# hse-cs/probaforms

Hardware: AMD Instinct MI355X
Metric: RealNVP samples/sec (fit+sample) (higher is better)
Workload: dtype f32 (first Linear of the s/t nets on 3-term split-bf16 MFMA, float32-level accuracy in: the training kernel's forward phase, sampling, log-prob; everything else f32); 1 GPU; C2: RealNVP n=1000000/GPU d=16 cond=4 L=8 hidden=(128,); one step = one fit epoch over the rank's 1000000 rows (16 batches of 65536 rows per rank incl. the ragged one: loss+grad+Adam each) + sampling 1000000 rows (counter-based prior draw inside the inverse kernel); global_batch=65536, rank_batch=65536, batch_mode=per-rank batch fixed (default): the global batch grows with N, parallelism=dp1, rccl_ranks=0

## Files before the change

### probaforms_amd/csrc/rnvp_mfma_layer.h

```cpp
#pragma once
#include "rnvp_mfma.h"

namespace rnvp {
namespace mfma {

using f4 = __attribute__((ext_vector_type(4))) float;

__device__ __forceinline__ f4 mfma16(float a, float b, f4 c) {
    return __builtin_amdgcn_mfma_f32_16x16x4f32(a, b, c, 0, 0, 0);
}

__device__ __forceinline__ f4 mfma4(float a, float b, f4 c) {
    return __builtin_amdgcn_mfma_f32_4x4x1f32(a, b, c, 0, 0, 0);
}

__device__ __forceinline__ float swap_add32(float x, float y) {
    const auto r = __builtin_amdgcn_permlane32_swap(__float_as_uint(x), __float_as_uint(y), false, false);
    return __uint_as_float(r[0]) + __uint_as_float(r[1]);
}
__device__ __forceinline__ float swap_add16(float x, float y) {
    const auto r = __builtin_amdgcn_permlane16_swap(__float_as_uint(x), __float_as_uint(y), false, false);
    return __uint_as_float(r[0]) + __uint_as_float(r[1]);
}

#ifndef RNVP_ABLATE
#define RNVP_ABLATE 0
#endif
#ifdef RNVP_NO_X4
constexpr bool kUseX4 = false;
#else
constexpr bool kUseX4 = true;
#endif

constexpr float kTanhScale = 2.8853900817779268f;
using f2 = __attribute__((ext_vector_type(2))) float;

__device__ __forceinline__ f4 tanh4(f4 u) {
    if (RNVP_ABLATE & 8) return u * 0.5f;
    f2 e0, e1;
    e0[0] = __builtin_amdgcn_exp2f(u[0]); e0[1] = __builtin_amdgcn_exp2f(u[1]);
    e1[0] = __builtin_amdgcn_exp2f(u[2]); e1[1] = __builtin_amdgcn_exp2f(u[3]);
    e0 = e0 + 1.0f; e1 = e1 + 1.0f;
    f2 r0, r1;
    r0[0] = __builtin_amdgcn_rcpf(e0[0]); r0[1] = __builtin_amdgcn_rcpf(e0[1]);
    r1[0] = __builtin_amdgcn_rcpf(e1[0]); r1[1] = __builtin_amdgcn_rcpf(e1[1]);
    r0 = __builtin_elementwise_fma(r0, f2{-2.0f, -2.0f}, f2{1.0f, 1.0f});
    r1 = __builtin_elementwise_fma(r1, f2{-2.0f, -2.0f}, f2{1.0f, 1.0f});
    return f4{r0[0], r0[1], r1[0], r1[1]};
}

template <int ACT> __device__ __forceinline__ f4 act4(f4 u) {
    if constexpr (ACT == 0) return tanh4(u);
    return f4{fmaxf(u[0], 0.f), fmaxf(u[1], 0.f), fmaxf(u[2], 0.f), fmaxf(u[3], 0.f)};
}
template <int ACT> __device__ __forceinline__ f4 dact4(f4 hv) {
    if constexpr (ACT == 0) return 1.0f - hv * hv;
    return f4{hv[0] > 0.f ? 1.f : 0.f, hv[1] > 0.f ? 1.f : 0.f, hv[2] > 0.f ? 1.f : 0.f, hv[3] > 0.f ? 1.f : 0.f};
}

typedef const __attribute__((address_space(1))) f4 *gf4_ptr;
__device__ __forceinline__ gf4_ptr opaque(const float *p) {
    asm volatile("" : "+v"(p));
    return (gf4_ptr)p;
}

template <int NF, int CQ, bool WITH_X = true>
__device__ __forceinline__ void load_row(const float *x, const float *__restrict__ c, int64_t src,
                                         int d, int cd, bool full, int q, float (&xr)[2 * NF],
                                         float (&cr)[CQ > 0 ? CQ : 1]) {
    if (full) {
        if constexpr (WITH_X) {
            const float *xp = x + src * (8 * NF) + q * 2 * NF;
#pragma unroll
            for (int v = 0; v < 2 * NF; v += 4) {
                const f4 t = *reinterpret_cast<const f4 *>(xp + v);
                xr[v] = t[0]; xr[v + 1] = t[1]; xr[v + 2] = t[2]; xr[v + 3] = t[3];
            }
        }
        if (CQ > 0) {
            const float *cp = c + src * (4 * CQ) + q * CQ;
#pragma unroll
            for (int v = 0; v < CQ; ++v) cr[v] = cp[v];
        } else {
            cr[0] = 0.f;
        }
    } else {
        if constexpr (WITH_X) {
#pragma unroll
            for (int v = 0; v < 2 * NF; ++v) {
                const int j = q * 2 * NF + v;
                xr[v] = (j < d) ? x[src * d + j] : 0.f;
            }
        }
#pragma unroll
        for (int v = 0; v < (CQ > 0 ? CQ : 1); ++v) {
            const int j = q * CQ + v;
            cr[v] = (CQ > 0 && j < cd) ? c[src * cd + j] : 0.f;
        }
    }
}

template <int NF>
__device__ __forceinline__ void store_row(float *out, int64_t row, int d, bool full, int q, const float (&xr)[2 * NF]) {
    if (full) {
        float *op = out + row * (8 * NF) + q * 2 * NF;
#pragma unroll
        for (int v = 0; v < 2 * NF; v += 4) {
            f4 t;
            t[0] = xr[v]; t[1] = xr[v + 1]; t[2] = xr[v + 2]; t[3] = xr[v + 3];
            *reinterpret_cast<f4 *>(op + v) = t;
        }
    } else {
#pragma unroll
        for (int v = 0; v < 2 * NF; ++v) {
            const int j = q * 2 * NF + v;
            if (j < d) out[row * d + j] = xr[v];
// ... 185 lines not shown
    }
    auto gemm2 = [&](const St &c, const f4 (&hv)[R]) {
#pragma unroll
        for (int o = 0; o < OTL; ++o)
#pragma unroll
            for (int rho = 0; rho < 4; ++rho)
#pragma unroll
                for (int rt = 0; rt < R; ++rt) out[rt][OT0 + o] = mfma16(c.a2c[o][rho], hv[rt][rho], out[rt][OT0 + o]);
    };
    auto step = [&](const St &c, St &nx, int t) {
        const int t2 = (t + 2 < last) ? t + 2 : last;
#pragma unroll
        for (int k4 = 0; k4 < K4; ++k4) nx.a1n[k4] = *opaque(pA1 + ((size_t)t2 * K4 + k4) * 256);
        nx.b1n = *opaque(pB1 + t2 * 16);
#pragma unroll
        for (int o = 0; o < OTL; ++o) nx.a2c[o] = *opaque(pA2 + ((size_t)(t + 1) * OTL + o) * 256);
        __builtin_amdgcn_sched_barrier(0);
        f4 hv[R];
        constexpr int RB = (R % 2 == 0) ? 2 : 1;
#pragma unroll
        for (int r0 = 0; r0 < R; r0 += RB) {
#pragma unroll
            for (int u = 0; u < RB; ++u) nx.acc[r0 + u] = c.b1n;
            if constexpr (BX) {
#pragma unroll
                for (int i = 0; i < K4; ++i)
#pragma unroll
                    for (int u = 0; u < RB; ++u) nx.acc[r0 + u] = mfma32(c.a1n[i], bin[r0 + u][i], nx.acc[r0 + u]);
            } else {
#pragma unroll
                for (int kk = 0; kk < NF + CQ; ++kk)
#pragma unroll
                    for (int u = 0; u < RB; ++u)
                        nx.acc[r0 + u] = mfma16(c.a1n[kk >> 2][kk & 3], in_op<NF, CQ, PC, R>(xr, cr, r0 + u, kk), nx.acc[r0 + u]);
            }
#pragma unroll
            for (int u = 0; u < RB; ++u) hv[r0 + u] = act4<ACT>(c.acc[r0 + u]);
            __builtin_amdgcn_sched_barrier(0);
        }
        gemm2(c, hv);
        __builtin_amdgcn_sched_barrier(0);
    };
    auto finish = [&](const St &c) {
        f4 hv[R];
#pragma unroll
        for (int rt = 0; rt < R; ++rt) hv[rt] = act4<ACT>(c.acc[rt]);
        gemm2(c, hv);
    };
    int t = 0;
    for (; t + 1 < last; t += 2) { step(s0, s1, t); step(s1, s0, t + 1); }
    if (t < last) { step(s0, s1, t); finish(s1); } else finish(s0);
}

template <int CQ, int R, int PC, int NET, int ACT, bool BX = false>
__device__ __forceinline__ void run_tiles_x4(const float *__restrict__ W, const Geo &g, int lane, int tile0,
                                             int ntiles, const float (&xr)[R][4],
                                             const float (&cr)[R][CQ > 0 ? CQ : 1], f4 (&outx)[R][4],
                                             const f4 (*bin)[SplitDims<2, CQ>::NI1] = nullptr,
                                             const TilePre<2, CQ> *pre = nullptr) {
    constexpr int NF = 2;
    constexpr int K4 = G1Dims<NF, CQ, BX>::NA;
    const int q = lane >> 4;
    const float *pA1 = W + (BX ? g.oA1S : g.oA1) + ((size_t)tile0 * K4 * 64 + lane) * 4;
    const float *pB1 = W + g.oB1 + ((size_t)tile0 * 4 + q) * 4;
    const float *pA2 = W + g.oA2X + ((size_t)tile0 * 2 * 64 + lane) * 4;
    const int last = ntiles - 1;
    struct St { f4 a1n[K4], b1n, a2c[2], acc[R]; };
    St s0, s1;
    {
        f4 a1c[K4], b1c;
        bool have = false;
        if constexpr (!BX) {
            if (pre) {
                have = true;
#pragma unroll
                for (int k4 = 0; k4 < K4; ++k4) { a1c[k4] = pre->a1c[k4]; s0.a1n[k4] = pre->a1n[k4]; }
                b1c = pre->b1c; s0.b1n = pre->b1n;
                s0.a2c[0] = pre->a2c[0]; s0.a2c[1] = pre->a2c[1];
            }
        }
        if (!have) {
#pragma unroll
        for (int k4 = 0; k4 < K4; ++k4) a1c[k4] = *reinterpret_cast<const f4 *>(pA1 + k4 * 256);
        b1c = *reinterpret_cast<const f4 *>(pB1);
#pragma unroll
        for (int o = 0; o < 2; ++o) s0.a2c[o] = *reinterpret_cast<const f4 *>(pA2 + o * 256);
        const int t1 = last < 1 ? last : 1;
#pragma unroll
        for (int k4 = 0; k4 < K4; ++k4) s0.a1n[k4] = *opaque(pA1 + ((size_t)t1 * K4 + k4) * 256);
        s0.b1n = *opaque(pB1 + t1 * 16);
        }
#pragma unroll
        for (int rt = 0; rt < R; ++rt) s0.acc[rt] = gemm1_any<NF, CQ, PC, R, BX>(a1c, b1c, xr, cr, bin, rt);
    }
    auto gemm2 = [&](const St &c, const f4 (&hv)[R]) {
#pragma unroll
        for (int rho = 0; rho < 4; ++rho)
#pragma unroll
            for (int o = 0; o < 2; ++o)
#pragma unroll
                for (int rt = 0; rt < R; ++rt)
                    outx[rt][2 * NET + o] = mfma4(c.a2c[o][rho], hv[rt][rho], outx[rt][2 * NET + o]);
    };
    auto step = [&](const St &c, St &nx, int t) {
        const int t2 = (t + 2 < last) ? t + 2 : last;
#pragma unroll
        for (int k4 = 0; k4 < K4; ++k4) nx.a1n[k4] = *opaque(pA1 + ((size_t)t2 * K4 + k4) * 256);
        nx.b1n = *opaque(pB1 + t2 * 16);
#pragma unroll
        for (int o = 0; o < 2; ++o) nx.a2c[o] = *opaque(pA2 + ((size_t)(t + 1) * 2 + o) * 256);
        __builtin_amdgcn_sched_barrier(0);
        f4 hv[R];
        constexpr int RB = (R % 2 == 0) ? 2 : 1;
#pragma unroll
        for (int r0 = 0; r0 < R; r0 += RB) {
#pragma unroll
            for (int u = 0; u < RB; ++u) nx.acc[r0 + u] = c.b1n;
            if constexpr (BX) {
#pragma unroll
                for (int i = 0; i < K4; ++i)
#pragma unroll
                    for (int u = 0; u < RB; ++u) nx.acc[r0 + u] = mfma32(c.a1n[i], bin[r0 + u][i], nx.acc[r0 + u]);
            } else {
#pragma unroll
                for (int kk = 0; kk < NF + CQ; ++kk)
#pragma unroll
                    for (int u = 0; u < RB; ++u)
                        nx.acc[r0 + u] = mfma16(c.a1n[kk >> 2][kk & 3], in_op<NF, CQ, PC, R>(xr, cr, r0 + u, kk), nx.acc[r0 + u]);
            }
#pragma unroll
            for (int u = 0; u < RB; ++u) hv[r0 + u] = act4<ACT>(c.acc[r0 + u]);
            __builtin_amdgcn_sched_barrier(0);
        }
        gemm2(c, hv);
        __builtin_amdgcn_sched_barrier(0);
    };
    auto finish = [&](const St &c) {
        f4 hv[R];
#pragma unroll
        for (int rt = 0; rt < R; ++rt) hv[rt] = act4<ACT>(c.acc[rt]);
        gemm2(c, hv);
    };
    int t = 0;
    for (; t + 1 < last; t += 2) { step(s0, s1, t); step(s1, s0, t + 1); }
    if (t < last) { step(s0, s1, t); finish(s1); } else finish(s0);
}

__device__ __forceinline__ void reduce_scatter_x4(const f4 (&part)[4], float (&tv)[2], float (&sv)[2]) {
#pragma unroll
    for (int net = 0; net < 2; ++net) {
        float s4[4];
#pragma unroll
        for (int i = 0; i < 4; ++i) s4[i] = swap_add32(part[2 * net][i], part[2 * net + 1][i]);
        const float f0 = swap_add16(s4[0], s4[2]), f1 = swap_add16(s4[1], s4[3]);
        if (net == 0) { tv[0] = f0; tv[1] = f1; } else { sv[0] = f0; sv[1] = f1; }
    }
}

template <int NF, int CQ, int R, int PC, int MODE, int ACT, bool BX = false>
__device__ __forceinline__ void layer_forward(const float *__restrict__ W, const Geo &g, int lane,
                                              float (&xr)[R][2 * NF], const float (&cr)[R][CQ > 0 ? CQ : 1],
                                              float (&ld)[R], float *__restrict__ scr) {
    using D = FwdDims<NF, CQ>;
// ... 15 lines not shown
        for (int rt = 0; rt < R; ++rt) {
            float tv[2], sv[2];
            reduce_scatter_x4(outx[rt], tv, sv);
            out[rt][0] = f4{tv[0], tv[1], sv[0], sv[1]} + bias2;
        }
    } else {
#pragma unroll
        for (int ot = 0; ot < NT2; ++ot) {
            const f4 b = (ot == 0) ? bias2 : *reinterpret_cast<const f4 *>(W + g.oB2 + (ot * 4 + q) * 4);
#pragma unroll
            for (int rt = 0; rt < R; ++rt) out[rt][ot] = b;
        }
        if (NF >= 4) {
            run_tiles<NF, CQ, R, PC, 0, ACT, BX>(W, g, lane, 0, g.HT, xr, cr, out, bin);
            run_tiles<NF, CQ, R, PC, (NF >= 4 ? OTL : 0), ACT, BX>(W, g, lane, g.HT, g.HT, xr, cr, out, bin);
        } else {
            run_tiles<NF, CQ, R, PC, 0, ACT, BX>(W, g, lane, 0, 2 * g.HT, xr, cr, out, bin);
        }
    }
#pragma unroll
    for (int rt = 0; rt < R; ++rt) {
#pragma unroll
        for (int f = 0; f < NF; ++f) {
            float tv, sv;
            if (NF >= 4) { tv = out[rt][f >> 2][f & 3]; sv = out[rt][(NF >= 4 ? OTL : 0) + (f >> 2)][f & 3]; }
            else { tv = out[rt][0][f & 1]; sv = out[rt][0][2 + (f & 1)]; }
            const int e = 2 * f + 1 - PC;
            if (MODE == 1) {
                xr[rt][e] = (xr[rt][e] - tv) * expf(-sv);
            } else {
                const float es = expf(sv), xv = xr[rt][e];
                if (MODE == 2) {
                    scr[((rt * 2 * NF) + f) * 64 + lane] = xv;
                    scr[((rt * 2 * NF) + NF + f) * 64 + lane] = es;
                }
                xr[rt][e] = fmaf(xv, es, tv);
                ld[rt] += sv;
            }
        }
    }
}

template <int NF, int CQ, int R, int PC, int MODE, int ACT, bool BX = false>
__device__ __forceinline__ void layer_forward_ns(const float *__restrict__ W, const Geo &g, int lane, int role,
                                                 float *xown, const float *xother, float (&xr)[R][2 * NF],
                                                 const float (&cr)[R][CQ > 0 ? CQ : 1], float (&ld)[R],
                                                 float *__restrict__ scr) {
    using D = FwdDims<NF, CQ>;
    constexpr int OTL = D::OTL, NT2 = D::NT2;
    const int q = lane >> 4;
    f4 bin[BX ? R : 1][SplitDims<NF, CQ>::NI1];
    if constexpr (BX) build_bin<NF, CQ, PC, R>(xr, cr, bin);
    float own[R][NF];
    if constexpr (NF == 2 && kUseX4) {
        const f4 bias2 = *reinterpret_cast<const f4 *>(W + g.oB2 + q * 4);
        f4 outx[R][4];
#pragma unroll
        for (int rt = 0; rt < R; ++rt)
#pragma unroll
            for (int u = 0; u < 4; ++u) outx[rt][u] = f4{0.f, 0.f, 0.f, 0.f};
        if (role == 0) {
            run_tiles_x4<CQ, R, PC, 0, ACT, BX>(W, g, lane, 0, g.HT, xr, cr, outx, bin);
#pragma unroll
            for (int rt = 0; rt < R; ++rt) {
                float s4[4];
#pragma unroll
                for (int i = 0; i < 4; ++i) s4[i] = swap_add32(outx[rt][0][i], outx[rt][1][i]);
                own[rt][0] = swap_add16(s4[0], s4[2]) + bias2[0];
                own[rt][1] = swap_add16(s4[1], s4[3]) + bias2[1];
            }
        } else {
            run_tiles_x4<CQ, R, PC, 1, ACT, BX>(W, g, lane, g.HT, g.HT, xr, cr, outx, bin);
#pragma unroll
            for (int rt = 0; rt < R; ++rt) {
                float s4[4];
#pragma unroll
                for (int i = 0; i < 4; ++i) s4[i] = swap_add32(outx[rt][2][i], outx[rt][3][i]);
                own[rt][0] = swap_add16(s4[0], s4[2]) + bias2[2];
                own[rt][1] = swap_add16(s4[1], s4[3]) + bias2[3];
            }
        }
    } else {
        f4 out[R][NT2];
#pragma unroll
        for (int ot = 0; ot < NT2; ++ot) {
            const f4 b = *reinterpret_cast<const f4 *>(W + g.oB2 + (ot * 4 + q) * 4);
#pragma unroll
            for (int rt = 0; rt < R; ++rt) out[rt][ot] = b;
        }
        if (role == 0) {
            run_tiles<NF, CQ, R, PC, 0, ACT, BX>(W, g, lane, 0, g.HT, xr, cr, out, bin);
#pragma unroll
            for (int rt = 0; rt < R; ++rt)
#pragma unroll
                for (int f = 0; f < NF; ++f) own[rt][f] = out[rt][f >> 2][f & 3];
        } else {
            run_tiles<NF, CQ, R, PC, (NF >= 4 ? OTL : 0), ACT, BX>(W, g, lane, g.HT, g.HT, xr, cr, out, bin);
#pragma unroll
            for (int rt = 0; rt < R; ++rt)
#pragma unroll
                for (int f = 0; f < NF; ++f) own[rt][f] = out[rt][(NF >= 4 ? OTL : 0) + (f >> 2)][(f & 3) + (NF >= 4 ? 0 : 2)];
        }
    }
#pragma unroll
    for (int rt = 0; rt < R; ++rt)
#pragma unroll
        for (int f = 0; f < NF; ++f) xown[(rt * NF + f) * 64 + lane] = own[rt][f];
    __syncthreads();
#pragma unroll
    for (int rt = 0; rt < R; ++rt) {
#pragma unroll
        for (int f = 0; f < NF; ++f) {
            const float oth = xother[(rt * NF + f) * 64 + lane];
            const float tv = role == 0 ? own[rt][f] : oth, sv = role == 0 ? oth : own[rt][f];
            const int e = 2 * f + 1 - PC;
            if (MODE == 1) {
                xr[rt][e] = (xr[rt][e] - tv) * expf(-sv);
            } else {
                const float es = expf(sv), xv = xr[rt][e];
                if (MODE == 2) {
                    if (role == 0) scr[((rt * 2 * NF) + f) * 64 + lane] = xv;
                    else scr[((rt * 2 * NF) + NF + f) * 64 + lane] = es;
                }
                xr[rt][e] = fmaf(xv, es, tv);
                ld[rt] += sv;
            }
        }
    }
}

constexpr int kTsWaves = 8, kTsSlices = 4;
template <int NF, int CQ, int R, int PC, int MODE, int ACT>
__device__ __forceinline__ void layer_forward_ts(const float *__restrict__ W, const Geo &g, int lane, int wave, int tile0,
                                                 int nt, float *red, float (&xr)[R][2 * NF],
                                                 const float (&cr)[R][CQ > 0 ? CQ : 1], float (&ld)[R],
                                                 float *__restrict__ scr, const float *__restrict__ Wnext,
                                                 TilePre<NF, CQ> &pre, bool use_pre) {
    using D = FwdDims<NF, CQ>;
    constexpr int OTL = D::OTL, NT2 = D::NT2;
    const int q = lane >> 4, net = wave >> 2;
    float b2t[NF], b2s[NF];
#pragma unroll
    for (int f = 0; f < NF; ++f) {
        if (NF >= 4) {
            b2t[f] = W[g.oB2 + ((f >> 2) * 4 + q) * 4 + (f & 3)];
            b2s[f] = W[g.oB2 + ((OTL + (f >> 2)) * 4 + q) * 4 + (f & 3)];
        } else {
            b2t[f] = W[g.oB2 + q * 4 + (f & 1)];
            b2s[f] = W[g.oB2 + q * 4 + 2 + (f & 1)];
        }
    }
    float own[R][NF];
    if constexpr (NF == 2 && kUseX4) {
        f4 outx[R][4];
#pragma unroll
        for (int rt = 0; rt < R; ++rt)
#pragma unroll
            for (int u = 0; u < 4; ++u) outx[rt][u] = f4{0.f, 0.f, 0.f, 0.f};
        if (nt > 0) {
            if (net == 0) run_tiles_x4<CQ, R, PC, 0, ACT>(W, g, lane, tile0, nt, xr, cr, outx, nullptr, use_pre ? &pre : nullptr);
            else run_tiles_x4<CQ, R, PC, 1, ACT>(W, g, lane, g.HT + tile0, nt, xr, cr, outx, nullptr, use_pre ? &pre : nullptr);
// ... 63 lines not shown
```

### probaforms_amd/csrc/rnvp_mfma_train_dev.h

```cpp
#pragma once
#include <atomic>

#include "rnvp_mfma_layer.h"

#ifndef RNVP_WPE
#define RNVP_WPE 2
#endif

namespace rnvp {
namespace mfma {

struct TrainPlan {
    int glayer_floats;
    size_t lds_bytes;
    int RMAX;
    size_t scratch_per_wave;
};
struct PartialLayout { int glayer_floats, w2c; };

namespace {

constexpr int kAblate = RNVP_ABLATE;
#ifdef RNVP_STAMP
#define STAMP(var) do { __builtin_amdgcn_sched_barrier(0); var = __builtin_readcyclecounter(); __builtin_amdgcn_sched_barrier(0); } while (0)
// ... 62 lines not shown
        return (w2c<NS>() ? gimg<NS>(R) : NT2 * 16 * kTS) + 16 * SIN + 2 * (R >= 4 ? 2 : R) * 16 * kTS;
    }
};

template <int NF, int CQ, int R> struct BwdPre {
    static constexpr int K4 = Dims<NF, CQ>::K4, OTL = Dims<NF, CQ>::OTL, NGI = (NF == 2 && kUseX4) ? 2 : Dims<NF, CQ>::MTI;
    float sx[R][NF], se[R][NF];
    f4 a1[K4], b1, a2t[OTL], a1t[NGI];
};
template <int NF, int CQ, int R>
__device__ __forceinline__ void load_bwd_pre(const float *__restrict__ W, const Geo &g, int lane, const float *__restrict__ scr,
                                             int net, int ht_lo, BwdPre<NF, CQ, R> &p) {
    using P = BwdPre<NF, CQ, R>;
    constexpr int K4 = P::K4, OTL = P::OTL, NGI = P::NGI;
    constexpr bool X4 = (NF == 2) && kUseX4;
    const int q = lane >> 4, HT = g.HT;
#pragma unroll
    for (int rt = 0; rt < R; ++rt)
#pragma unroll
        for (int f = 0; f < NF; ++f) {
            p.sx[rt][f] = scr[((rt * 2 * NF) + f) * 64 + lane];
            p.se[rt][f] = scr[((rt * 2 * NF) + NF + f) * 64 + lane];
        }
    const float *pA1 = W + g.oA1 + ((size_t)net * HT * K4 * 64 + lane) * 4;
    const float *pB1 = W + g.oB1 + ((size_t)net * HT * 4 + q) * 4;
    const float *pA2T = W + g.oA2T + ((size_t)net * HT * OTL * 64 + lane) * 4;
    const float *pA1T = W + (X4 ? g.oA1X : g.oA1T) + ((size_t)net * HT * NGI * 64 + lane) * 4;
#pragma unroll
    for (int k4 = 0; k4 < K4; ++k4) p.a1[k4] = *opaque(pA1 + ((size_t)ht_lo * K4 + k4) * 256);
    p.b1 = *opaque(pB1 + ht_lo * 16);
#pragma unroll
    for (int o = 0; o < OTL; ++o) p.a2t[o] = *opaque(pA2T + ((size_t)ht_lo * OTL + o) * 256);
#pragma unroll
    for (int m = 0; m < NGI; ++m) p.a1t[m] = *opaque(pA1T + ((size_t)ht_lo * NGI + m) * 256);
}

template <int NF, int CQ, int R, int PC, int NS, int ACT, int WV = kWaves>
__device__ __forceinline__ void layer_bwd(const float *__restrict__ W, const Geo &g, int lane, int wave,
                                          float (&xr)[R][2 * NF], const float (&cr)[R][CQ > 0 ? CQ : 1],
                                          float (&gy)[R][2 * NF], const float (&gld)[R],
                                          const float *__restrict__ scr, float *lds, float *tb,
                                          float *gp_layer, bool first, Stamps &stp, float *xown,
                                          const float *xother, int tile_lo, int tile_hi,
                                          BwdPre<NF, CQ, R> &pre_ref, bool use_pre, const float *__restrict__ Wprev = nullptr,
                                          const float *__restrict__ scr_prev = nullptr, FlushSync *fs = nullptr) {
    BwdPre<NF, CQ, R> *const pre = &pre_ref;
    constexpr bool TS = NS == 2;
    unsigned long long t0 = 0; (void)t0;
    STAMP(t0);
    using D = Dims<NF, CQ>;
    constexpr int KS1 = D::KS1, K4 = D::K4, OTL = D::OTL, NT2 = D::NT2, KP4 = D::KP4, NTI = D::NTI,
                  MTI = D::MTI, KSP = D::KSP, SIN = D::SIN;
    const int q = lane >> 4, r = lane & 15, tid = wave * 64 + lane;
    const int role = NS ? (wave >> 2) : 0;
    const int HT = g.HT;
    const int ht_lo = TS ? tile_lo : 0, ht_hi = TS ? tile_hi : HT;
    constexpr bool W2C = D::template w2c<NS>();
    constexpr int FT = D::FT, SLOT = D::template slot<NS>(), TBLK = D::template tblk<NS>(), GS = D::GS;
    constexpr bool TFW = kWideTFlush && NS == 0 && WV == 8 && FT >= 2 && FT % 2 == 0;
    constexpr bool TF = (kNsTFlush && NS == 1 && FT >= 2 && FT % 2 == 0 && WV == 4) || TFW;
    constexpr int FT2 = FT / 2 > 0 ? FT / 2 : 1;
    const int netblock = HT * TBLK;
    float *slot = lds + wave * SLOT;
    float *bufG = tb;
    float *bufI = tb + (W2C ? D::template gimg<NS>(R) : NT2 * 16 * kTS);
    float *bufH = bufI + 16 * SIN;
    f4 go[R][NT2];
#pragma unroll
    for (int rt = 0; rt < R; ++rt) {
#pragma unroll
        for (int f = 0; f < NF; ++f) {
            const float sx = (TS && use_pre) ? pre->sx[rt][f] : scr[((rt * 2 * NF) + f) * 64 + lane];
            const float se = (TS && use_pre) ? pre->se[rt][f] : scr[((rt * 2 * NF) + NF + f) * 64 + lane];
            const int e = 2 * f + 1 - PC;
            const float gyv = gy[rt][e];
            const float gt = gyv;
            const float gs = fmaf(gyv * sx, se, gld[rt]);
            gy[rt][e] = gyv * se;
            xr[rt][e] = sx;
            if (NF >= 4) { go[rt][f >> 2][f & 3] = gt; go[rt][(NF >= 4 ? OTL : 0) + (f >> 2)][f & 3] = gs; }
            else { go[rt][0][f & 1] = gt; go[rt][0][2 + (f & 1)] = gs; }
        }
    }
    f4 gb2[NT2];
#pragma unroll
    for (int ot = 0; ot < NT2; ++ot) {
        gb2[ot] = go[0][ot];
#pragma unroll
        for (int rt = 1; rt < R; ++rt) gb2[ot] += go[rt][ot];
    }
    float goT[R][NT2][4], inT[R][NTI][4];
#pragma unroll
    for (int rt = 0; rt < R; ++rt) {
        if constexpr (W2C && NS == 0) {
            float *gp = bufG + (rt * 16 + r) * GS + 4 * (q & 1) + (q >> 1);
            wave_lds_fence();
            gp[0] = go[rt][0][0]; gp[2] = go[rt][0][1];
            gp[R * 16 * GS] = go[rt][0][2]; gp[R * 16 * GS + 2] = go[rt][0][3];
        } else if constexpr (W2C) {
            const float v0 = role ? go[rt][0][2] : go[rt][0][0], v1 = role ? go[rt][0][3] : go[rt][0][1];
            float *gp = bufG + (rt * 16 + r) * GS + 4 * (q & 1) + (q >> 1);
            wave_lds_fence();
            gp[0] = v0; gp[2] = v1;
        } else {
#pragma unroll
            for (int ot = 0; ot < NT2; ++ot) transpose16(bufG + ot * 16 * kTS, go[rt][ot], lane, goT[rt][ot]);
        }
        wave_lds_fence();
#pragma unroll
        for (int k4 = 0; k4 < KP4; ++k4) {
            f4 v;
#pragma unroll
            for (int u = 0; u < 4; ++u) {
                const int kk = 4 * k4 + u;
                v[u] = (kk < KS1) ? in_op<NF, CQ, PC, R>(xr, cr, rt, kk < KS1 ? kk : 0)
                                  : (kk == KS1 ? (q == 0 ? 1.0f : 0.0f) : 0.0f);
            }
            *reinterpret_cast<f4 *>(bufI + r * SIN + q * KSP + 4 * k4) = v;
        }
        wave_lds_fence();
#pragma unroll
        for (int nt = 0; nt < NTI; ++nt)
#pragma unroll
            for (int ks = 0; ks < 4; ++ks) inT[rt][nt][ks] = bufI[(4 * ks + q) * SIN + 16 * nt + r];
    }
    constexpr bool X4 = (NF == 2) && kUseX4;
    constexpr int NGI = X4 ? 2 : MTI;
    f4 gin[R][NGI];
#pragma unroll
    for (int rt = 0; rt < R; ++rt)
#pragma unroll
        for (int mt = 0; mt < NGI; ++mt) gin[rt][mt] = f4{0.f, 0.f, 0.f, 0.f};
    STAMP_ADD(stp.bsetup, t0);

    auto net_pass = [&](auto net_c) {
        constexpr int net = decltype(net_c)::value;
        const float *pA1 = W + g.oA1 + ((size_t)net * HT * K4 * 64 + lane) * 4;
        const float *pB1 = W + g.oB1 + ((size_t)net * HT * 4 + q) * 4;
        const float *pA2T = W + g.oA2T + ((size_t)net * HT * OTL * 64 + lane) * 4;
        const float *pA1T = W + (X4 ? g.oA1X : g.oA1T) + ((size_t)net * HT * NGI * 64 + lane) * 4;
        f4 a1[K4], a2t[OTL], a1t[NGI], b1;
        bool have = false;
        if constexpr (TS) {
            if (use_pre) {
                have = true;
#pragma unroll
                for (int k4 = 0; k4 < K4; ++k4) a1[k4] = pre->a1[k4];
                b1 = pre->b1;
#pragma unroll
                for (int o = 0; o < OTL; ++o) a2t[o] = pre->a2t[o];
#pragma unroll
                for (int m = 0; m < NGI; ++m) a1t[m] = pre->a1t[m];
            }
        }
        if (!have) {
#pragma unroll
        for (int k4 = 0; k4 < K4; ++k4) a1[k4] = *reinterpret_cast<const f4 *>(pA1 + ((size_t)ht_lo * K4 + k4) * 256);
        b1 = *reinterpret_cast<const f4 *>(pB1 + ht_lo * 16);
#pragma unroll
        for (int o = 0; o < OTL; ++o) a2t[o] = *reinterpret_cast<const f4 *>(pA2T + ((size_t)ht_lo * OTL + o) * 256);
#pragma unroll
        for (int m = 0; m < NGI; ++m) a1t[m] = *reinterpret_cast<const f4 *>(pA1T + ((size_t)ht_lo * NGI + m) * 256);
        }
        for (int ht = ht_lo; ht < ht_hi; ++ht) {
            const int nx = (kAblate & 64) ? 0 : ((ht + 1 < ht_hi) ? ht + 1 : ht);
            constexpr bool INPL = NF >= 4;
            f4 na1[K4], na2t[OTL], na1t[NGI], nb1;
            if constexpr (!INPL) {
#pragma unroll
                for (int k4 = 0; k4 < K4; ++k4) na1[k4] = *opaque(pA1 + ((size_t)nx * K4 + k4) * 256);
                nb1 = *opaque(pB1 + nx * 16);
#pragma unroll
                for (int o = 0; o < OTL; ++o) na2t[o] = *opaque(pA2T + ((size_t)nx * OTL + o) * 256);
#pragma unroll
                for (int m = 0; m < NGI; ++m) na1t[m] = *opaque(pA1T + ((size_t)nx * NGI + m) * 256);
            }
            BWD_SCHED_BARRIER();

            f4 gW2[W2C ? 2 : OTL], gW1[NTI];
#pragma unroll
            for (int o = 0; o < (W2C ? 2 : OTL); ++o) gW2[o] = f4{0.f, 0.f, 0.f, 0.f};
#pragma unroll
            for (int nt = 0; nt < NTI; ++nt) gW1[nt] = f4{0.f, 0.f, 0.f, 0.f};
            constexpr int RH = (R >= 4) ? 2 : R;
#pragma unroll
            for (int r0 = 0; r0 < R; r0 += RH) {
                f4 acc[RH], gh[RH];
#pragma unroll
                for (int u = 0; u < RH; ++u) { acc[u] = b1; gh[u] = f4{0.f, 0.f, 0.f, 0.f}; }
#pragma unroll
                for (int kk = 0; kk < KS1; ++kk)
#pragma unroll
                    for (int u = 0; u < RH; ++u)
                        acc[u] = mfma16(a1[kk >> 2][kk & 3], in_op<NF, CQ, PC, R>(xr, cr, r0 + u, kk), acc[u]);
                if (NF >= 4) {
#pragma unroll
                    for (int o = 0; o < OTL; ++o)
#pragma unroll
                        for (int rho = 0; rho < 4; ++rho)
#pragma unroll
                            for (int u = 0; u < RH; ++u)
                                gh[u] = mfma16(a2t[o][rho], go[r0 + u][(NF >= 4 ? net * OTL : 0) + o][rho], gh[u]);
                } else {
#pragma unroll
                    for (int v = 0; v < 2; ++v)
#pragma unroll
                        for (int u = 0; u < RH; ++u)
                            gh[u] = mfma16(a2t[0][2 * net + v], go[r0 + u][0][2 * net + v], gh[u]);
                }
                if constexpr (INPL) {
                    if (r0 + RH >= R) {
#pragma unroll
                        for (int k4 = 0; k4 < K4; ++k4) a1[k4] = *opaque(pA1 + ((size_t)nx * K4 + k4) * 256);
                        b1 = *opaque(pB1 + nx * 16);
#pragma unroll
                        for (int o = 0; o < OTL; ++o) a2t[o] = *opaque(pA2T + ((size_t)nx * OTL + o) * 256);
                    }
                }
                BWD_SCHED_BARRIER();
                STAMP_ADD(stp.p1, t0);

                f4 gpv[RH];
                wave_lds_fence();
#pragma unroll
                for (int u = 0; u < RH; ++u) {
                    const f4 hv = act4<ACT>(acc[u]);
                    gpv[u] = gh[u] * dact4<ACT>(hv);
                    if (!(kAblate & 1)) {
                        *reinterpret_cast<f4 *>(bufH + (2 * u) * 16 * kTS + r * kTS + 4 * q) = hv;
                        *reinterpret_cast<f4 *>(bufH + (2 * u + 1) * 16 * kTS + r * kTS + 4 * q) = gpv[u];
                    } else {
                        asm volatile("" ::"v"(hv));
                    }
                }
                wave_lds_fence();
                BWD_SCHED_BARRIER();
                STAMP_ADD(stp.p2, t0);

                float hT[RH][4], pT[RH][4];
                float2 gB[W2C ? RH : 1][4];
                auto read_transposed = [&]() {
#pragma unroll
                    for (int u = 0; u < RH; ++u)
#pragma unroll
                        for (int ks = 0; ks < 4; ++ks) {
                            if (!(kAblate & 1)) {
                                hT[u][ks] = bufH[(2 * u) * 16 * kTS + (4 * ks + q) * kTS + r];
                                pT[u][ks] = bufH[(2 * u + 1) * 16 * kTS + (4 * ks + q) * kTS + r];
                            } else {
                                hT[u][ks] = gpv[u][ks]; pT[u][ks] = gpv[u][ks];
                            }
                            if constexpr (W2C)
                                gB[u][ks] = *reinterpret_cast<const float2 *>(bufG + (NS == 0 ? net * R * 16 * GS : 0) +
                                                                              ((r0 + u) * 16 + 4 * ks + q) * GS + 2 * (r & 3));
                        }
                };
                if constexpr (X4) {
#pragma unroll
                    for (int rho = 0; rho < 4; ++rho)
#pragma unroll
                        for (int m = 0; m < 2; ++m)
#pragma unroll
                            for (int u = 0; u < RH; ++u) gin[r0 + u][m] = mfma4(a1t[m][rho], gpv[u][rho], gin[r0 + u][m]);
                } else {
#pragma unroll
                    for (int m = 0; m < MTI; ++m)
#pragma unroll
                        for (int rho = 0; rho < 4; ++rho)
#pragma unroll
                            for (int u = 0; u < RH; ++u)
                                gin[r0 + u][m] = mfma16(a1t[m][rho], gpv[u][rho], gin[r0 + u][m]);
                }
                if constexpr (INPL) {
                    if (r0 + RH >= R) {
#pragma unroll
                        for (int m = 0; m < NGI; ++m) a1t[m] = *opaque(pA1T + ((size_t)nx * NGI + m) * 256);
                    }
                }
                read_transposed();
                BWD_SCHED_BARRIER();
                STAMP_ADD(stp.p3, t0);

                if (!(kAblate & 32)) {
#pragma unroll
                    for (int u = 0; u < RH; ++u)
#pragma unroll
                        for (int ks = 0; ks < 4; ++ks) {
                            if constexpr (W2C) {
                                gW2[0] = mfma4(hT[u][ks], gB[u][ks].x, gW2[0]);
                                gW2[1] = mfma4(hT[u][ks], gB[u][ks].y, gW2[1]);
                            } else {
#pragma unroll
                                for (int o = 0; o < OTL; ++o)
                                    gW2[o] = mfma16(hT[u][ks], goT[r0 + u][(NF >= 4 ? net * OTL : 0) + o][ks], gW2[o]);
                            }
#pragma unroll
                            for (int nt = 0; nt < NTI; ++nt) gW1[nt] = mfma16(pT[u][ks], inT[r0 + u][nt][ks], gW1[nt]);
                        }
// ... 213 lines not shown
            gi[rt][1] = swap_add16(s4[1], s4[3]);
        } else {
#pragma unroll
            for (int f = 0; f < NF; ++f) gi[rt][f] = (NF >= 4) ? gin[rt][f >> 2][f & 3] : gin[rt][0][f & 1];
        }
    }
    if constexpr (TS) {
#pragma unroll
        for (int rt = 0; rt < R; ++rt)
#pragma unroll
            for (int f = 0; f < NF; ++f) xown[(rt * NF + f) * 64 + lane] = gi[rt][f];
        __syncthreads();
#pragma unroll
        for (int rt = 0; rt < R; ++rt)
#pragma unroll
            for (int f = 0; f < NF; ++f) {
                float a = 0.f;
#pragma unroll
                for (int w = 0; w < kTsWaves; ++w) a += xother[(w * R * NF + rt * NF + f) * 64 + lane];
                gi[rt][f] = a;
            }
    } else if constexpr (NS) {
#pragma unroll
        for (int rt = 0; rt < R; ++rt)
#pragma unroll
            for (int f = 0; f < NF; ++f) xown[(rt * NF + f) * 64 + lane] = gi[rt][f];
        __syncthreads();
#pragma unroll
        for (int rt = 0; rt < R; ++rt)
#pragma unroll
            for (int f = 0; f < NF; ++f) {
                const float o = xother[(rt * NF + f) * 64 + lane];
                gi[rt][f] = role == 0 ? gi[rt][f] + o : o + gi[rt][f];
            }
    }
#pragma unroll
    for (int rt = 0; rt < R; ++rt) {
#pragma unroll
        for (int f = 0; f < NF; ++f) gy[rt][2 * f + PC] += gi[rt][f];
    }
    STAMP_ADD(stp.btail, t0);
}

template <int NF, int CQ, int R, int NS, int ACT, bool BXF, int WV = kWaves>
__device__ __forceinline__ void train_body(const float *__restrict__ wp, const Geo &g, int L, int alt, const float *__restrict__ x,
             const float *__restrict__ c, const int64_t *__restrict__ row_index, int64_t n, float inv_B,
             float *gpart, float *losspart, float *scratch, int glayer_floats, Seeds sd) {
    using DM = Dims<NF, CQ>;
    constexpr int D = 8 * NF, CD = 4 * CQ;
    constexpr int NW = WV * (1 + NS);
    constexpr int XW = R * NF * 64;
    extern __shared__ __attribute__((aligned(16))) float lds[];
    const int lane = threadIdx.x & 63, wave = threadIdx.x >> 6;
    const int pw = wave & (WV - 1), role = NS ? wave >> 2 : 0;
    const int q = lane >> 4, r = lane & 15;
    constexpr int SLOTN = DM::template slot<NS>(), TBN = DM::template tbn<R, NS>();
    float *tb = lds + NW * SLOTN + wave * TBN;
    float *xbuf = lds + NW * SLOTN + NW * TBN;
    int *sync = reinterpret_cast<int *>(xbuf + (NS ? 2 * NW * XW : 0));
    const Poison poison{losspart + (size_t)blockIdx.x * kWaves, sync + 13, error_word(losspart)};
    FlushSync fsync{sync + 8, sync + 12, 0, poison};
    if constexpr (NS == 1 || (kWideTFlush && NS == 0 && WV == 8)) {
        if (threadIdx.x < 6) sync[8 + threadIdx.x] = 0;
        __syncthreads();
    }
    const int64_t rows_per_wg = (int64_t)WV * R * 16;
    const int64_t ngroups = (n + rows_per_wg - 1) / rows_per_wg;
    const float prior_c = 0.5f * (float)g.d * kLog2Pi;
    const bool full = (g.d == D) && (g.c == CD) && ((uintptr_t)x & 15) == 0;
    float *gp = gpart + (size_t)blockIdx.x * glayer_floats * L;
    float *scr_wave = scratch + ((size_t)blockIdx.x * WV + pw) * L * R * 2 * NF * 64;
    float wave_sum = 0.f;
    bool first = true;
    Stamps stp = {0, 0, 0, 0, 0, 0, 0, 0, 0, 0, 0, 0, 0};
    unsigned long long t0 = 0, tk0 = 0; (void)t0; (void)tk0;
    STAMP(tk0);
    for (int64_t grp = blockIdx.x; grp < ngroups; grp += gridDim.x) {
        STAMP(t0);
        const int64_t base = grp * rows_per_wg + (int64_t)pw * R * 16;
        float xr[R][2 * NF], cr[R][CQ > 0 ? CQ : 1], ld[R], gy[R][2 * NF], gld[R];
        bool valid[R];
#pragma unroll
        for (int rt = 0; rt < R; ++rt) {
            const int64_t row = base + rt * 16 + r;
            valid[rt] = row < n;
            const int64_t src = valid[rt] ? (row_index ? row_index[row] : row) : 0;
            load_row<NF, CQ>(x, c, src, g.d, g.c, full, q, xr[rt], cr[rt]);
            ld[rt] = 0.f;
        }
        STAMP_ADD(stp.ld, t0);
        for (int l = 0; l < L; ++l) {
            const float *W = wp + (size_t)l * g.layer_floats;
            float *scr = scr_wave + (size_t)l * R * 2 * NF * 64;
            if constexpr (NS) {
                float *xb = xbuf + (size_t)(l & 1) * NW * XW;
                if ((l + alt) & 1) layer_forward_ns<NF, CQ, R, 1, 2, ACT, BXF>(W, g, lane, role, xb + wave * XW, xb + (wave ^ WV) * XW, xr, cr, ld, scr);
                else layer_forward_ns<NF, CQ, R, 0, 2, ACT, BXF>(W, g, lane, role, xb + wave * XW, xb + (wave ^ WV) * XW, xr, cr, ld, scr);
            } else {
                if ((l + alt) & 1) layer_forward<NF, CQ, R, 1, 2, ACT, BXF>(W, g, lane, xr, cr, ld, scr);
                else layer_forward<NF, CQ, R, 0, 2, ACT, BXF>(W, g, lane, xr, cr, ld, scr);
            }
        }
        if constexpr (NS) __syncthreads();
#pragma unroll
        for (int rt = 0; rt < R; ++rt) {
            float ss = 0.f;
#pragma unroll
// ... 374 lines not shown
```

Measured before the change: 397.8 million rows/s.

## Use scalar-base weight loads, per-role accumulators, and precomputed LDS bases in net-split training

```diff
diff --git a/probaforms_amd/csrc/rnvp_mfma_layer.h b/probaforms_amd/csrc/rnvp_mfma_layer.h
--- a/probaforms_amd/csrc/rnvp_mfma_layer.h
+++ b/probaforms_amd/csrc/rnvp_mfma_layer.h
@@ -1,4 +1,6 @@
 #pragma once
+#include <type_traits>
+
 #include "rnvp_mfma.h"
 
 namespace rnvp {
@@ -31,6 +33,17 @@
 #else
 constexpr bool kUseX4 = true;
 #endif
+
+#ifndef RNVP_NS_SADDR
+#define RNVP_NS_SADDR 1
+#endif
+#ifndef RNVP_NS_OWNACC
+#define RNVP_NS_OWNACC 1
+#endif
+#ifndef RNVP_NS_LDSBASE
+#define RNVP_NS_LDSBASE 1
+#endif
+constexpr bool kNsSaddr = RNVP_NS_SADDR != 0, kNsOwnAcc = RNVP_NS_OWNACC != 0, kNsLdsBase = RNVP_NS_LDSBASE != 0;
 
 constexpr float kTanhScale = 2.8853900817779268f;
 using f2 = __attribute__((ext_vector_type(2))) float;
@@ -62,6 +75,19 @@
 __device__ __forceinline__ gf4_ptr opaque(const float *p) {
     asm volatile("" : "+v"(p));
     return (gf4_ptr)p;
+}
+
+typedef const __attribute__((address_space(1))) float *gw_ptr;
+__device__ __forceinline__ gw_ptr sbase_w(const float *p) {
+    asm volatile("" : "+s"(p));
+    return (gw_ptr)p;
+}
+__device__ __forceinline__ f4 gl_w4(gw_ptr base, unsigned off) { return *reinterpret_cast<const __attribute__((address_space(1))) f4 *>(base + off); }
+typedef __attribute__((address_space(3))) float *lds_ptr;
+__device__ __forceinline__ lds_ptr lds_base(float *p) {
+    lds_ptr l = (lds_ptr)p;
+    asm volatile("" : "+v"(l));
+    return l;
 }
 
 template <int NF, int CQ, bool WITH_X = true>
@@ -353,10 +379,10 @@
     if (t < last) { step(s0, s1, t); finish(s1); } else finish(s0);
 }
 
-template <int CQ, int R, int PC, int NET, int ACT, bool BX = false>
+template <int CQ, int R, int PC, int NET, int ACT, bool BX = false, int NO = 4, bool SB = false>
 __device__ __forceinline__ void run_tiles_x4(const float *__restrict__ W, const Geo &g, int lane, int tile0,
                                              int ntiles, const float (&xr)[R][4],
-                                             const float (&cr)[R][CQ > 0 ? CQ : 1], f4 (&outx)[R][4],
+                                             const float (&cr)[R][CQ > 0 ? CQ : 1], f4 (&outx)[R][NO],
                                              const f4 (*bin)[SplitDims<2, CQ>::NI1] = nullptr,
                                              const TilePre<2, CQ> *pre = nullptr) {
     constexpr int NF = 2;
@@ -365,13 +391,30 @@
     const float *pA1 = W + (BX ? g.oA1S : g.oA1) + ((size_t)tile0 * K4 * 64 + lane) * 4;
     const float *pB1 = W + g.oB1 + ((size_t)tile0 * 4 + q) * 4;
     const float *pA2 = W + g.oA2X + ((size_t)tile0 * 2 * 64 + lane) * 4;
+    const float *uA1 = W + (BX ? g.oA1S : g.oA1) + (size_t)tile0 * K4 * 256, *uB1 = W + g.oB1 + (size_t)tile0 * 16;
+    const float *uA2 = W + g.oA2X + (size_t)tile0 * 2 * 256;
+    const unsigned lo4 = lane * 4, qo4 = q * 4;
     const int last = ntiles - 1;
     struct St { f4 a1n[K4], b1n, a2c[2], acc[R]; };
     St s0, s1;
     {
         f4 a1c[K4], b1c;
         bool have = false;
-        if constexpr (!BX) {
+        if constexpr (SB) {
+            have = true;
+            const int t1 = last < 1 ? last : 1;
+            const gw_ptr g1 = sbase_w(uA1), gb = sbase_w(uB1), g2 = sbase_w(uA2);
+            const gw_ptr g1n = sbase_w(uA1 + (size_t)t1 * K4 * 256), gbn = sbase_w(uB1 + t1 * 16);
+#pragma unroll
+            for (int k4 = 0; k4 < K4; ++k4) a1c[k4] = gl_w4(g1, lo4 + k4 * 256);
+            b1c = gl_w4(gb, qo4);
+#pragma unroll
+            for (int o = 0; o < 2; ++o) s0.a2c[o] = gl_w4(g2, lo4 + o * 256);
+#pragma unroll
+            for (int k4 = 0; k4 < K4; ++k4) s0.a1n[k4] = gl_w4(g1n, lo4 + k4 * 256);
+            s0.b1n = gl_w4(gbn, qo4);
+        }
+        if constexpr (!BX && !SB) {
             if (pre) {
                 have = true;
 #pragma unroll
@@ -405,11 +448,21 @@
     };
     auto step = [&](const St &c, St &nx, int t) {
         const int t2 = (t + 2 < last) ? t + 2 : last;
+        if constexpr (SB) {
+            const gw_ptr g1 = sbase_w(uA1 + (size_t)t2 * K4 * 256), gb = sbase_w(uB1 + t2 * 16);
+            const gw_ptr g2 = sbase_w(uA2 + (size_t)(t + 1) * 2 * 256);
+#pragma unroll
+            for (int k4 = 0; k4 < K4; ++k4) nx.a1n[k4] = gl_w4(g1, lo4 + k4 * 256);
+            nx.b1n = gl_w4(gb, qo4);
+#pragma unroll
+            for (int o = 0; o < 2; ++o) nx.a2c[o] = gl_w4(g2, lo4 + o * 256);
+        } else {
 #pragma unroll
         for (int k4 = 0; k4 < K4; ++k4) nx.a1n[k4] = *opaque(pA1 + ((size_t)t2 * K4 + k4) * 256);
         nx.b1n = *opaque(pB1 + t2 * 16);
 #pragma unroll
         for (int o = 0; o < 2; ++o) nx.a2c[o] = *opaque(pA2 + ((size_t)(t + 1) * 2 + o) * 256);
+        }
         __builtin_amdgcn_sched_barrier(0);
         f4 hv[R];
         constexpr int RB = (R % 2 == 0) ? 2 : 1;
@@ -531,7 +584,24 @@
     f4 bin[BX ? R : 1][SplitDims<NF, CQ>::NI1];
     if constexpr (BX) build_bin<NF, CQ, PC, R>(xr, cr, bin);
     float own[R][NF];
-    if constexpr (NF == 2 && kUseX4) {
+    if constexpr (NF == 2 && kUseX4 && kNsOwnAcc) {
+        const float *b2 = W + g.oB2 + q * 4 + 2 * role;
+        const float bias0 = b2[0], bias1 = b2[1];
+        f4 outx[R][2];
+#pragma unroll
+        for (int rt = 0; rt < R; ++rt)
+#pragma unroll
+            for (int u = 0; u < 2; ++u) outx[rt][u] = f4{0.f, 0.f, 0.f, 0.f};
+        run_tiles_x4<CQ, R, PC, 0, ACT, BX, 2, kNsSaddr>(W, g, lane, role * g.HT, g.HT, xr, cr, outx, bin);
+#pragma unroll
+        for (int rt = 0; rt < R; ++rt) {
+            float s4[4];
+#pragma unroll
+            for (int i = 0; i < 4; ++i) s4[i] = swap_add32(outx[rt][0][i], outx[rt][1][i]);
+            own[rt][0] = swap_add16(s4[0], s4[2]) + bias0;
+            own[rt][1] = swap_add16(s4[1], s4[3]) + bias1;
+        }
+    } else if constexpr (NF == 2 && kUseX4) {
         const f4 bias2 = *reinterpret_cast<const f4 *>(W + g.oB2 + q * 4);
         f4 outx[R][4];
 #pragma unroll
@@ -539,7 +609,7 @@
 #pragma unroll
             for (int u = 0; u < 4; ++u) outx[rt][u] = f4{0.f, 0.f, 0.f, 0.f};
         if (role == 0) {
-            run_tiles_x4<CQ, R, PC, 0, ACT, BX>(W, g, lane, 0, g.HT, xr, cr, outx, bin);
+            run_tiles_x4<CQ, R, PC, 0, ACT, BX, 4, kNsSaddr>(W, g, lane, 0, g.HT, xr, cr, outx, bin);
 #pragma unroll
             for (int rt = 0; rt < R; ++rt) {
                 float s4[4];
@@ -549,7 +619,7 @@
                 own[rt][1] = swap_add16(s4[1], s4[3]) + bias2[1];
             }
         } else {
-            run_tiles_x4<CQ, R, PC, 1, ACT, BX>(W, g, lane, g.HT, g.HT, xr, cr, outx, bin);
+            run_tiles_x4<CQ, R, PC, 1, ACT, BX, 4, kNsSaddr>(W, g, lane, g.HT, g.HT, xr, cr, outx, bin);
 #pragma unroll
             for (int rt = 0; rt < R; ++rt) {
                 float s4[4];
@@ -586,6 +656,30 @@
 #pragma unroll
         for (int f = 0; f < NF; ++f) xown[(rt * NF + f) * 64 + lane] = own[rt][f];
     __syncthreads();
+    if constexpr (NF == 2 && kUseX4 && kNsOwnAcc) {
+        static_assert(MODE == 2, "the net-split layer serves the training kernel");
+        float oth[R][NF];
+#pragma unroll
+        for (int rt = 0; rt < R; ++rt)
+#pragma unroll
+            for (int f = 0; f < NF; ++f) oth[rt][f] = xother[(rt * NF + f) * 64 + lane];
+        auto couple = [&](const float (&tva)[R][NF], const float (&sva)[R][NF], float *rec, auto is_t) {
+#pragma unroll
+            for (int rt = 0; rt < R; ++rt)
+#pragma unroll
+                for (int f = 0; f < NF; ++f) {
+                    const float tv = tva[rt][f], sv = sva[rt][f];
+                    const int e = 2 * f + 1 - PC;
+                    const float es = expf(sv), xv = xr[rt][e];
+                    rec[((rt * 2 * NF) + f) * 64] = decltype(is_t)::value ? xv : es;
+                    xr[rt][e] = fmaf(xv, es, tv);
+                    ld[rt] += sv;
+                }
+        };
+        if (role == 0) couple(own, oth, scr + lane, std::true_type{});
+        else couple(oth, own, scr + NF * 64 + lane, std::false_type{});
+        return;
+    }
 #pragma unroll
     for (int rt = 0; rt < R; ++rt) {
 #pragma unroll
diff --git a/probaforms_amd/csrc/rnvp_mfma_train_dev.h b/probaforms_amd/csrc/rnvp_mfma_train_dev.h
--- a/probaforms_amd/csrc/rnvp_mfma_train_dev.h
+++ b/probaforms_amd/csrc/rnvp_mfma_train_dev.h
@@ -138,7 +138,8 @@
     constexpr int KS1 = D::KS1, K4 = D::K4, OTL = D::OTL, NT2 = D::NT2, KP4 = D::KP4, NTI = D::NTI,
                   MTI = D::MTI, KSP = D::KSP, SIN = D::SIN;
     const int q = lane >> 4, r = lane & 15, tid = wave * 64 + lane;
-    const int role = NS ? (wave >> 2) : 0;
+    constexpr bool SB = NF == 2 && NS == 1 && kNsSaddr;
+    const int role = NS ? (SB ? __builtin_amdgcn_readfirstlane(wave >> 2) : (wave >> 2)) : 0;
     const int HT = g.HT;
     const int ht_lo = TS ? tile_lo : 0, ht_hi = TS ? tile_hi : HT;
     constexpr bool W2C = D::template w2c<NS>();
@@ -219,14 +220,38 @@
         for (int mt = 0; mt < NGI; ++mt) gin[rt][mt] = f4{0.f, 0.f, 0.f, 0.f};
     STAMP_ADD(stp.bsetup, t0);
 
+    constexpr bool LB = NF == 2 && NS == 1 && W2C && kNsLdsBase && !(kAblate & 1);
+    constexpr int RHL = (R >= 4) ? 2 : R;
+    lds_ptr hrd[2 * RHL], grd[R / RHL];
+    if constexpr (LB) {
+#pragma unroll
+        for (int t = 0; t < 2 * RHL; ++t) hrd[t] = lds_base(bufH + t * 16 * kTS + q * kTS + r);
+#pragma unroll
+        for (int h = 0; h < R / RHL; ++h) grd[h] = lds_base(bufG + (h * RHL * 16 + q) * GS + 2 * (r & 3));
+    }
     auto net_pass = [&](auto net_c) {
         constexpr int net = decltype(net_c)::value;
         const float *pA1 = W + g.oA1 + ((size_t)net * HT * K4 * 64 + lane) * 4;
         const float *pB1 = W + g.oB1 + ((size_t)net * HT * 4 + q) * 4;
         const float *pA2T = W + g.oA2T + ((size_t)net * HT * OTL * 64 + lane) * 4;
         const float *pA1T = W + (X4 ? g.oA1X : g.oA1T) + ((size_t)net * HT * NGI * 64 + lane) * 4;
+        const float *uA1 = W + g.oA1 + (size_t)net * HT * K4 * 256, *uB1 = W + g.oB1 + (size_t)net * HT * 16;
+        const float *uA2T = W + g.oA2T + (size_t)net * HT * OTL * 256, *uA1T = W + (X4 ? g.oA1X : g.oA1T) + (size_t)net * HT * NGI * 256;
+        const unsigned lo4 = lane * 4, qo4 = q * 4;
         f4 a1[K4], a2t[OTL], a1t[NGI], b1;
         bool have = false;
+        if constexpr (SB) {
+            have = true;
+            const gw_ptr s1 = sbase_w(uA1 + (size_t)ht_lo * K4 * 256), sb = sbase_w(uB1 + ht_lo * 16);
+            const gw_ptr s2 = sbase_w(uA2T + (size_t)ht_lo * OTL * 256), s3 = sbase_w(uA1T + (size_t)ht_lo * NGI * 256);
+#pragma unroll
+            for (int k4 = 0; k4 < K4; ++k4) a1[k4] = gl_w4(s1, lo4 + k4 * 256);
+            b1 = gl_w4(sb, qo4);
+#pragma unroll
+            for (int o = 0; o < OTL; ++o) a2t[o] = gl_w4(s2, lo4 + o * 256);
+#pragma unroll
+            for (int m = 0; m < NGI; ++m) a1t[m] = gl_w4(s3, lo4 + m * 256);
+        }
         if constexpr (TS) {
             if (use_pre) {
                 have = true;
@@ -252,7 +277,17 @@
             const int nx = (kAblate & 64) ? 0 : ((ht + 1 < ht_hi) ? ht + 1 : ht);
             constexpr bool INPL = NF >= 4;
             f4 na1[K4], na2t[OTL], na1t[NGI], nb1;
-            if constexpr (!INPL) {
+            if constexpr (SB) {
+                const gw_ptr s1 = sbase_w(uA1 + (size_t)nx * K4 * 256), sb = sbase_w(uB1 + nx * 16);
+                const gw_ptr s2 = sbase_w(uA2T + (size_t)nx * OTL * 256), s3 = sbase_w(uA1T + (size_t)nx * NGI * 256);
+#pragma unroll
+                for (int k4 = 0; k4 < K4; ++k4) na1[k4] = gl_w4(s1, lo4 + k4 * 256);
+                nb1 = gl_w4(sb, qo4);
+#pragma unroll
+                for (int o = 0; o < OTL; ++o) na2t[o] = gl_w4(s2, lo4 + o * 256);
+#pragma unroll
+                for (int m = 0; m < NGI; ++m) na1t[m] = gl_w4(s3, lo4 + m * 256);
+            } else if constexpr (!INPL) {
 #pragma unroll
                 for (int k4 = 0; k4 < K4; ++k4) na1[k4] = *opaque(pA1 + ((size_t)nx * K4 + k4) * 256);
                 nb1 = *opaque(pB1 + nx * 16);
@@ -330,6 +365,13 @@
                     for (int u = 0; u < RH; ++u)
 #pragma unroll
                         for (int ks = 0; ks < 4; ++ks) {
+                            if constexpr (LB) {
+                                hT[u][ks] = hrd[2 * u][4 * ks * kTS];
+                                pT[u][ks] = hrd[2 * u + 1][4 * ks * kTS];
+                                const f2 gv = *reinterpret_cast<const __attribute__((address_space(3))) f2 *>(grd[r0 / RH] + (u * 16 + 4 * ks) * GS);
+                                gB[u][ks].x = gv[0]; gB[u][ks].y = gv[1];
+                                continue;
+                            }
                             if (!(kAblate & 1)) {
                                 hT[u][ks] = bufH[(2 * u) * 16 * kTS + (4 * ks + q) * kTS + r];
                                 pT[u][ks] = bufH[(2 * u + 1) * 16 * kTS + (4 * ks + q) * kTS + r];
@@ -649,7 +691,8 @@
     constexpr int XW = R * NF * 64;
     extern __shared__ __attribute__((aligned(16))) float lds[];
     const int lane = threadIdx.x & 63, wave = threadIdx.x >> 6;
-    const int pw = wave & (WV - 1), role = NS ? wave >> 2 : 0;
+    constexpr bool SROLE = NS == 1 && NF == 2 && (kNsSaddr || kNsOwnAcc);
+    const int pw = wave & (WV - 1), role = NS ? (SROLE ? __builtin_amdgcn_readfirstlane(wave >> 2) : wave >> 2) : 0;
     const int q = lane >> 4, r = lane & 15;
     constexpr int SLOTN = DM::template slot<NS>(), TBN = DM::template tbn<R, NS>();
     float *tb = lds + NW * SLOTN + wave * TBN;
```

Result: faster. 426.7 million rows/s, median of 6 (+7.3%).
